# amplab/keystone

Measured on NVIDIA H100. Metric: block-LS fit samples/sec (N=1M, D=64K, k=1K), higher is better.
Workload: dtype f16x2

## Files before the change

### keystone_b200/build.py

```python
from __future__ import annotations

import os
import shutil
import subprocess
import sys

HERE = os.path.dirname(os.path.abspath(__file__))
CSRC = os.path.join(HERE, "csrc")
LIBDIR = os.path.join(HERE, "lib")
LIB = os.path.join(LIBDIR, "libkeystone_b200.so")
SOURCES = ["tc_kernels.cu", "aux_kernels.cu", "solve_kernels.cu", "engine.cu", "bwls.cu", "krr.cu", "lbfgs.cu", "sparse.cu", "logistic.cu", "pca.cu", "fisher.cu", "gmm_fit.cu", "sift.cu", "hog_daisy.cu", "augment.cu", "io.cu"]
HEADERS = ["tc_common.cuh", "kernels.h", "operand_split.cuh", "lbfgs_core.cuh", "engine.h", os.path.join("..", "..", "include", "keystone_b200.h")]
NVCC_FLAGS = [
    "-gencode", "arch=compute_90a,code=sm_90a", "-lineinfo", "-O3", "-std=c++17",
    "-Xcompiler", "-fPIC,-fvisibility=hidden", "-DKS_BUILD",
]


def _nvcc() -> str:
    for cand in (shutil.which("nvcc"), "/usr/local/cuda/bin/nvcc"):
        if cand and os.path.exists(cand):
            return cand
    raise RuntimeError("nvcc not found")


def _stale(target: str, deps) -> bool:
    if not os.path.exists(target):
# ... 31 lines not shown
```

### keystone_b200/csrc/engine.cu

```cuda
#include "engine.h"

#include <cuda_fp16.h>
#include <dlfcn.h>
#include <stdlib.h>
#include <math.h>
#include <string.h>

#include <chrono>
#include <functional>
#include <mutex>
#include <sstream>

namespace ks {

template <class F>
static void load_sym(void* lib, const char* name, F& out, const char* libname) {
  void* s = dlsym(lib, name);
  if (!s) throw KsError{KS_ERR_SOLVER, std::string("symbol ") + name + " missing from " + libname};
  out = reinterpret_cast<F>(s);
}
static void* open_first(const std::vector<const char*>& names) {
  for (const char* n : names) {
    void* h = dlopen(n, RTLD_NOW | RTLD_GLOBAL);
    if (h) return h;
// ... 531 lines not shown
  k.p.vec1 = shift;
  k.p.colsum = colsum;
  k.p.colsumsq = colsumsq;
  k.p.M = static_cast<int>(rows);
  k.p.N = static_cast<int>(cols);
  k.p.K = static_cast<int>(kdepth);
  k.p.flags = (round_out ? 0 : KM_FLAG_NO_ROUND) | (src.kind == 1 ? KM_FLAG_RECT : 0);
  k.p.rect_floor = src.rect_floor;
  k.epi = EPI_COS;
  k.num_sms = (st == c.st2) ? std::max(1, c.num_sms - c.reserve_sms) : c.num_sms;
  if (c.dyn_tiles) k.p.tile_counter = c.next_tile_counter(st);
  KS_CUDA(launch_kmajor(k, st));
  c.launches += 1;
}

const GramTile* gram_tiles(Ctx& c, int b, int kcols, bool with_g, bool with_c, int* num_tiles) {
  std::vector<int> key = {b, kcols, with_g ? 1 : 0, with_c ? 1 : 0};
  auto it = c.tile_cache.find(key);
  std::vector<GramTile> t;
  const int tm = 128, tn = 128;
  const int mb = (b + tm - 1) / tm;
  if (with_g) {
    const int nbk = (b + tn - 1) / tn;
    for (int i = 0; i < mb; ++i)
      for (int j = 0; j < nbk; ++j)
        if ((j + 1) * tn - 1 >= i * tm) t.push_back(GramTile{i, j, 0, 0});
  }
  if (with_c) {
    const int nck = (kcols + tn - 1) / tn;
    for (int i = 0; i < mb; ++i)
      for (int j = 0; j < nck; ++j) t.push_back(GramTile{i, j, 1, 0});
  }
  *num_tiles = static_cast<int>(t.size());
  if (it != c.tile_cache.end()) return it->second->as<GramTile>();
  auto buf = std::make_unique<DevBuf>();
  buf->alloc(sizeof(GramTile) * std::max<size_t>(t.size(), 1));
  KS_CUDA(cudaMemcpyAsync(buf->p, t.data(), sizeof(GramTile) * t.size(), cudaMemcpyHostToDevice, c.st));
  KS_CUDA(cudaStreamSynchronize(c.st));
  const GramTile* p = buf->as<GramTile>();
  c.tile_cache[key] = std::move(buf);
  return p;
}

void launch_gram_block(Ctx& c, const void* slab, int64_t lds, int64_t rows, int b, const void* R, int64_t ldr, int kcols,
                       float* G, int ldg, float* C, int ldc, bool with_g, bool with_c, cudaStream_t st, bool f16,
                       int64_t chunk_rows, const void* slab_lo, const void* R_lo) {
  if (rows <= 0 || b <= 0 || (!with_g && !with_c)) return;
  if (!st) st = c.st;
  const bool split = slab_lo != nullptr;
  if (split && (!f16 || (with_c && !R_lo))) throw KsError{KS_ERR_INVALID, "split Gram operands must be fp16 pairs"};
  GramLaunch g;
  int nt = 0;
  g.f16 = f16 ? 1 : 0;
  g.split = split ? 1 : 0;
  g.tiles = gram_tiles(c, b, kcols, with_g, with_c, &nt);
  g.num_tiles = nt;
  const int stage_rows = split ? 32 : f16 ? 64 : kGramStageRows;
  if (f16) {
    tmap16_or_throw(&g.tmA, slab, rows, b, lds, 64, stage_rows, TMAP_SW128);
    g.tmB0 = g.tmA;
    if (with_c) tmap16_or_throw(&g.tmB1, R, rows, kcols, ldr, 64, stage_rows, TMAP_SW128);
    else g.tmB1 = g.tmA;
    if (split) {
      tmap16_or_throw(&g.tmAlo, slab_lo, rows, b, lds, 64, stage_rows, TMAP_SW128);
      g.tmB0lo = g.tmAlo;
      if (with_c) tmap16_or_throw(&g.tmB1lo, R_lo, rows, kcols, ldr, 64, stage_rows, TMAP_SW128);
      else g.tmB1lo = g.tmAlo;
    }
  } else {
    tmap_or_throw(&g.tmA, static_cast<const float*>(slab), rows, b, lds, kGramStageRows);
// ... 2191 lines not shown
```

### keystone_b200/csrc/engine.h

```cpp
#pragma once
#include <cuda_runtime.h>
#include <cusolverDn.h>
#include <nccl.h>
#include <stdint.h>

#include <map>
#include <memory>
#include <string>
#include <unordered_map>
#include <vector>

#include "../../include/keystone_b200.h"
#include "kernels.h"

namespace ks {

struct KsError {
  int code;
  std::string msg;
};

#define KS_CUDA(call)                                                                                   \
  do {                                                                                                  \
    cudaError_t e__ = (call);                                                                           \
// ... 276 lines not shown
  int64_t ldx3 = 0, ldw3 = 0;
  bool proj_x2 = false;
  DevBuf wcat, wcat_full, bcat;
  int64_t n_rows = 0;
  DevBuf zeros;
};
void make_feat_src(Ctx& c, int64_t features, int64_t x_in, const int64_t* rfs, int32_t n_rfs, FeatSrc& out,
                   int precision = 0);
void prepare_generated_operands(Ctx& c, FeatSrc& out, int precision);
void derive_feat_src(Ctx& c, const FeatSrc& src, Matrix* X, FeatSrc& out, int precision);
void produce_slab(Ctx& c, FeatSrc& src, int64_t c0, int64_t cols, const float* shift, void* slab, int64_t lds,
                  int64_t row_begin, int64_t rows, bool round_out = true, float* colsum = nullptr, cudaStream_t st = nullptr,
                  bool out16 = false, bool x2 = false,
                  void* slab_lo = nullptr,
                  double* colsumsq = nullptr);
const GramTile* gram_tiles(Ctx& c, int b, int kcols, bool with_g, bool with_c, int* num_tiles);
void launch_gram_block(Ctx& c, const void* slab, int64_t lds, int64_t rows, int b, const void* R, int64_t ldr, int kcols,
                       float* G, int ldg, float* C, int ldc, bool with_g, bool with_c, cudaStream_t st = nullptr,
                       bool f16 = false, int64_t chunk_rows = 0,
                       const void* slab_lo = nullptr, const void* R_lo = nullptr);
void launch_update(Ctx& c, const void* slab, int64_t lds, int64_t rows, int b, const void* bop, int64_t ldb, int k,
                   float* out, int64_t ldo, const float* cbias, int epi, bool reduce, cudaStream_t st = nullptr,
                   bool f16 = false, const float* acc_scale_ptr = nullptr,
                   const void* slab_lo = nullptr, const void* bop_lo = nullptr);

int64_t fit_bwls(Ctx& c, FeatSrc& src, Matrix& Y, int bs, int num_iter, double lam, double w, int64_t nf_opt,
                 int precision = KS_PRECISION_TF32);
void launch_set_f64(double* p, double v, cudaStream_t st);
void launch_scale_f64(const double* src, double scale, float* dst, double* dst64, int n, cudaStream_t st);
int64_t fit_lbfgs(Ctx& c, FeatSrc& src, Matrix& Y, bool fit_intercept, int num_corrections, double convergence_tol, int num_iterations,
                  double reg_param, int precision);
// ... 109 lines not shown
```

### keystone_b200/csrc/kernels.h

```cpp
#pragma once
#include <cuda.h>
#include <cuda_runtime.h>
#include <stdint.h>

namespace ks {

static constexpr int kGramStageRows = 32;
static constexpr int kPadCols = 32;

enum { EPI_COS = 0, EPI_UPDATE = 1, EPI_APPLY = 2, EPI_POOL = 3, EPI_RBF = 4 };

struct GramTile {
  int m_blk;
  int n_blk;
  int which;
  int pad;
};
struct GramLaunch {
  CUtensorMap tmA, tmB0, tmB1;
  CUtensorMap tmOut0, tmOut1;
  CUtensorMap tmAlo, tmB0lo, tmB1lo;
  const GramTile* tiles;
  int num_tiles;
  int rows;
  int chunk_rows;
  int n_valid0, n_valid1;
  int f16 = 0;
  int split = 0;
};
enum { KM_FLAG_NO_ROUND = 1, KM_FLAG_REDUCE = 2, KM_FLAG_RECT = 8 };
struct KmParams {
// ... 99 lines not shown
```

### keystone_b200/csrc/solve_kernels.cu

```cuda
#include "kernels.h"

namespace ks {

namespace {
constexpr int TS = 64;
constexpr int U = 16;

__device__ __forceinline__ void dmma(double (&d)[2], double a, double b) {
  asm volatile("mma.sync.aligned.m8n8k4.row.col.f64.f64.f64.f64 {%0, %1}, {%2}, {%3}, {%0, %1};"
               : "+d"(d[0]), "+d"(d[1])
               : "d"(a), "d"(b));
}

template <int NG, bool TRANS>
__device__ __forceinline__ void bulk_dmma(double (&acc)[NG][2], const double* __restrict__ Aptr, size_t lda, int mrow_limit,
                                          const double* Bptr, size_t ldb, const bool (&col_ok)[NG], int k0, int k1, int krow_limit,
                                          int lane) {
  const int m = lane >> 2, kq = lane & 3;
  const bool m_ok = m < mrow_limit;
  if (k0 >= k1) return;
  double a[U], an[U];
  auto load_a = [&](double (&dst)[U], int kb) {
#pragma unroll
    for (int u = 0; u < U; ++u) {
// ... 76 lines not shown
          for (int g = 0; g < NG; ++g) dmma(y[g], a, sV[kk * VP + 8 * g + m]);
        }
      }
#pragma unroll
      for (int g = 0; g < NG; ++g)
#pragma unroll
        for (int e = 0; e < 2; ++e) {
          const int row = r0 + m, col = c0 + 8 * g + 2 * cq + e;
          if (row < n && col < k) B[row + static_cast<size_t>(col) * ld] = y[g][e];
        }
      __syncthreads();
    }
  }
}

__device__ __forceinline__ uint32_t cl_ctarank() {
  uint32_t r;
  asm volatile("mov.u32 %0, %%cluster_ctarank;" : "=r"(r));
  return r;
}
__device__ __forceinline__ uint32_t cl_nctarank() {
  uint32_t r;
  asm volatile("mov.u32 %0, %%cluster_nctarank;" : "=r"(r));
  return r;
}
__device__ __forceinline__ void cl_sync() {
  asm volatile("barrier.cluster.arrive.release.aligned;" ::: "memory");
  asm volatile("barrier.cluster.wait.acquire.aligned;" ::: "memory");
}
__device__ __forceinline__ double ld_dsmem_f64(const double* local_ptr, uint32_t rank) {
  const uint32_t la = static_cast<uint32_t>(__cvta_generic_to_shared(local_ptr));
  uint32_t ra;
  asm("mapa.shared::cluster.u32 %0, %1, %2;" : "=r"(ra) : "r"(la), "r"(rank));
  double v;
  asm volatile("ld.shared::cluster.f64 %0, [%1];" : "=d"(v) : "r"(ra));
  return v;
}

template <bool TRANS>
__device__ __forceinline__ void bulk_dmma_cg(double (&acc)[2], const double* __restrict__ Aptr, size_t lda, int mrow_limit,
                                             const double* Bptr, size_t ldb, bool col_ok, int k0, int k1, int krow_limit, int lane) {
  const int m = lane >> 2, kq = lane & 3;
  const bool m_ok = m < mrow_limit;
  for (int kb = k0; kb < k1; kb += 4 * U) {
    double a[U], b[U];
#pragma unroll
    for (int u = 0; u < U; ++u) {
      const int kk = kb + 4 * u + kq;
// ... 144 lines not shown
```

### keystone_b200/csrc/tc_common.cuh

```cuda
#pragma once
#include <cuda.h>
#include <cuda_fp16.h>
#include <cuda_runtime.h>
#include <stdint.h>

namespace ks {

__device__ unsigned int g_wait_timeout_flag = 0;

static constexpr unsigned long long kWaitBudgetCycles = 6000000000ull;

__device__ __forceinline__ uint32_t smem_u32(const void* p) {
  return static_cast<uint32_t>(__cvta_generic_to_shared(p));
}

__device__ __forceinline__ bool elect_one() {
  uint32_t pred = 0;
  asm volatile(
      "{\n\t"
      ".reg .pred P;\n\t"
      "elect.sync _|P, 0xffffffff;\n\t"
      "selp.u32 %0, 1, 0, P;\n\t"
      "}\n"
      : "=r"(pred));
// ... 8 lines not shown
  asm volatile("mbarrier.init.shared::cta.b64 [%0], %1;" ::"r"(smem_u32(bar)), "r"(count));
}
__device__ __forceinline__ void fence_barrier_init() {
  asm volatile("fence.mbarrier_init.release.cluster;" ::: "memory");
}
__device__ __forceinline__ void fence_proxy_async() {
  asm volatile("fence.proxy.async.shared::cta;" ::: "memory");
}
__device__ __forceinline__ void mbar_arrive_expect_tx(uint64_t* bar, uint32_t bytes) {
  asm volatile("mbarrier.arrive.expect_tx.shared::cta.b64 _, [%0], %1;" ::"r"(smem_u32(bar)), "r"(bytes)
               : "memory");
}
__device__ __forceinline__ void mbar_arrive(uint64_t* bar) {
  asm volatile("mbarrier.arrive.shared::cta.b64 _, [%0];" ::"r"(smem_u32(bar)) : "memory");
}
__device__ __forceinline__ bool mbar_try_wait(uint64_t* bar, uint32_t parity) {
  uint32_t ok;
  asm volatile(
      "{\n\t"
      ".reg .pred P;\n\t"
      "mbarrier.try_wait.parity.shared::cta.b64 P, [%1], %2;\n\t"
      "selp.u32 %0, 1, 0, P;\n\t"
      "}\n"
      : "=r"(ok)
      : "r"(smem_u32(bar)), "r"(parity)
      : "memory");
  return ok != 0;
}
__device__ __forceinline__ void mbar_wait(uint64_t* bar, uint32_t parity) {
  if (mbar_try_wait(bar, parity)) return;
// ... 2 lines not shown
    if (clock64() - t0 > kWaitBudgetCycles) {
      atomicExch(&g_wait_timeout_flag, 1u + (blockIdx.x << 8) + (threadIdx.x >> 5));
      __trap();
    }
  }
}

__device__ __forceinline__ void tma_prefetch_desc(const CUtensorMap* m) {
  asm volatile("prefetch.tensormap [%0];" ::"l"(reinterpret_cast<uint64_t>(m)) : "memory");
}
__device__ __forceinline__ void tma_load_2d(void* smem_dst, const CUtensorMap* m, uint64_t* bar, int32_t c0,
                                            int32_t c1) {
  asm volatile(
      "cp.async.bulk.tensor.2d.shared::cluster.global.mbarrier::complete_tx::bytes [%0], [%1, {%3, %4}], [%2];"
      ::"r"(smem_u32(smem_dst)), "l"(reinterpret_cast<uint64_t>(m)), "r"(smem_u32(bar)), "r"(c0), "r"(c1)
      : "memory");
}

__device__ __forceinline__ void tma_store_2d(const CUtensorMap* m, const void* smem_src, int32_t c0, int32_t c1) {
  asm volatile("cp.async.bulk.tensor.2d.global.shared::cta.bulk_group [%0, {%2, %3}], [%1];" ::"l"(
                   reinterpret_cast<uint64_t>(m)),
               "r"(smem_u32(smem_src)), "r"(c0), "r"(c1)
               : "memory");
}
__device__ __forceinline__ void tma_reduce_add_2d(const CUtensorMap* m, const void* smem_src, int32_t c0, int32_t c1) {
  asm volatile("cp.reduce.async.bulk.tensor.2d.global.shared::cta.add.bulk_group [%0, {%2, %3}], [%1];" ::"l"(
                   reinterpret_cast<uint64_t>(m)),
               "r"(smem_u32(smem_src)), "r"(c0), "r"(c1)
               : "memory");
}
// ... 84 lines not shown
```

### keystone_b200/csrc/tc_kernels.cu

```cuda
#include <type_traits>

#include "tc_common.cuh"
#include "kernels.h"

namespace ks {

static constexpr int kThreads = 384;
static constexpr int kTileM = 128, kTileN = 128;
static constexpr int kStages = 4;
static constexpr int kRawLd = 65;
static constexpr int kRawBytes = 2 * 64 * kRawLd * 4;
static constexpr int kStagingBytes = 8 * 4096;
static constexpr int kVecBytes = 8 * 64 * 4;
static constexpr int kEpiBytes = kStagingBytes + kRawBytes + kVecBytes;
static constexpr int kStageBytes = 32768;
static constexpr int kSmemBytes = kStages * kStageBytes + kEpiBytes + 1024  + 256 ;
static_assert(kSmemBytes <= 227 * 1024, "shared memory per block");

struct SmemLayout {
  uint8_t* stages;
  uint8_t* staging;
  float* raw;
  float* vec;
  uint64_t* full_bar;
// ... 91 lines not shown
    named_bar_sync(1 + g, 128);
    chunk(o, slab, 32 * (w & 1), slab * 64 + 32 * (w >> 1));
  }
}

template <bool F16, bool SPLIT = false>
struct GramCfg {
  static constexpr int PLANES = SPLIT ? 4 : 2;
  static constexpr int SR = SPLIT ? 32 : F16 ? 64 : 32;
  static constexpr int CW = F16 ? 64 : 32;
  static constexpr int NBOX = kTileM / CW;
  static constexpr int BOX_BYTES = SR * 128;
  static constexpr int A_BYTES = NBOX * BOX_BYTES;
  static_assert(PLANES * A_BYTES == kStageBytes, "stage size");
  static_assert(!SPLIT || F16, "split operands are fp16 pairs");
};

template <int BOX_BYTES>
__device__ __forceinline__ uint32_t ld_mn_tf32(const uint8_t* tile, int c, int r) {
  return *reinterpret_cast<const uint32_t*>(tile + (c >> 5) * BOX_BYTES + r * 128 + (((((c & 31) >> 2) ^ (r & 7))) << 4) +
                                            ((c & 3) << 2));
}

template <bool F16, bool SPLIT>
__global__ void __launch_bounds__(kThreads, 1)
gram_tn_kernel(const __grid_constant__ CUtensorMap tmA, const __grid_constant__ CUtensorMap tmB0,
               const __grid_constant__ CUtensorMap tmB1, const __grid_constant__ CUtensorMap tmOut0,
               const __grid_constant__ CUtensorMap tmOut1, const __grid_constant__ CUtensorMap tmAlo,
               const __grid_constant__ CUtensorMap tmB0lo, const __grid_constant__ CUtensorMap tmB1lo,
               const GramTile* __restrict__ tiles, int num_tiles, int rows, int chunk_rows, int n_valid0, int n_valid1) {
  using Cfg = GramCfg<F16, SPLIT>;
  constexpr int SR = Cfg::SR;
  extern __shared__ uint8_t smem_raw[];
  const SmemLayout L = carve_smem(smem_raw);

  const int warp = threadIdx.x >> 5;
  const int lane = threadIdx.x & 31;
  const int wg = warp >> 2;
  const GramTile tile = tiles[blockIdx.x % num_tiles];
  const int chunk = blockIdx.x / num_tiles;
  const int row0 = chunk * chunk_rows;
  const int nrows = min(chunk_rows, rows - row0);
  const int ksteps = (nrows + SR - 1) / SR;
  const int m0 = tile.m_blk * kTileM;
  const int n0 = tile.n_blk * kTileN;
  const CUtensorMap* tmB = tile.which ? &tmB1 : &tmB0;
  const CUtensorMap* tmBlo = tile.which ? &tmB1lo : &tmB0lo;
  const CUtensorMap* tmOut = tile.which ? &tmOut1 : &tmOut0;

  if (threadIdx.x == 0) {
    tma_prefetch_desc(&tmA);
    tma_prefetch_desc(tmB);
    if (SPLIT) {
      tma_prefetch_desc(&tmAlo);
      tma_prefetch_desc(tmBlo);
    }
    tma_prefetch_desc(tmOut);
    for (int s = 0; s < kStages; ++s) {
      mbar_init(&L.full_bar[s], 1);
      mbar_init(&L.empty_bar[s], 8);
    }
    fence_barrier_init();
  }
  __syncthreads();

  if (wg == 0) {
    if (SPLIT) setmaxnreg_dec<40>();
    if (warp == 0 && elect_one()) {
      for (int ks = 0; ks < ksteps; ++ks) {
        const int s = ks % kStages;
        const uint32_t ph = (ks / kStages) & 1;
        mbar_wait(&L.empty_bar[s], ph ^ 1);
        mbar_arrive_expect_tx(&L.full_bar[s], kStageBytes);
        uint8_t* sA = L.stages + s * kStageBytes;
        const int r = row0 + ks * SR;
        const CUtensorMap* maps[4] = {&tmA, SPLIT ? &tmAlo : tmB, tmB, tmBlo};
#pragma unroll
        for (int pl = 0; pl < Cfg::PLANES; ++pl) {
          const int c0 = (pl < Cfg::PLANES / 2) ? m0 : n0;
#pragma unroll
          for (int i = 0; i < Cfg::NBOX; ++i)
            tma_load_2d(sA + pl * Cfg::A_BYTES + i * Cfg::BOX_BYTES, maps[pl], &L.full_bar[s], c0 + Cfg::CW * i, r);
        }
      }
    }
    return;
  }
  if (SPLIT) setmaxnreg_inc<232>();

  const int g = wg - 1;
  const int w = warp & 3;
  float acc[64];
#pragma unroll
  for (int i = 0; i < 64; ++i) acc[i] = 0.f;

  if (SPLIT) {
    float acc_x[64];
#pragma unroll
    for (int i = 0; i < 64; ++i) acc_x[i] = 0.f;
    wgmma_fence_acc(acc);
    wgmma_fence_acc(acc_x);
    int prev = -1;
    for (int ks = 0; ks < ksteps; ++ks) {
      const int s = ks % kStages;
      mbar_wait(&L.full_bar[s], (ks / kStages) & 1);
      const uint32_t st = smem_u32(L.stages + s * kStageBytes);
      const uint32_t sAhi = st + g * Cfg::BOX_BYTES, sAlo = sAhi + Cfg::A_BYTES;
      const uint32_t sBhi = st + 2 * Cfg::A_BYTES, sBlo = st + 3 * Cfg::A_BYTES;
      wgmma_fence();
#pragma unroll
      for (int kk = 0; kk < SR / 16; ++kk)
        wgmma_f16_n128<1, 1>(acc, make_wgmma_desc(sAhi + kk * 2048, Cfg::BOX_BYTES, 1024),
                             make_wgmma_desc(sBhi + kk * 2048, Cfg::BOX_BYTES, 1024), 1);
#pragma unroll
      for (int kk = 0; kk < SR / 16; ++kk) {
        wgmma_f16_n128<1, 1>(acc_x, make_wgmma_desc(sAlo + kk * 2048, Cfg::BOX_BYTES, 1024),
                             make_wgmma_desc(sBhi + kk * 2048, Cfg::BOX_BYTES, 1024), 1);
        wgmma_f16_n128<1, 1>(acc_x, make_wgmma_desc(sAhi + kk * 2048, Cfg::BOX_BYTES, 1024),
                             make_wgmma_desc(sBlo + kk * 2048, Cfg::BOX_BYTES, 1024), 1);
      }
      wgmma_commit();
      if (prev >= 0) {
        wgmma_wait<1>();
        if (lane == 0) mbar_arrive(&L.empty_bar[prev]);
      }
      prev = s;
    }
    wgmma_wait<0>();
    wgmma_fence_acc(acc);
    wgmma_fence_acc(acc_x);
#pragma unroll
    for (int i = 0; i < 64; ++i) acc[i] = __fadd_rn(acc[i], acc_x[i]);
  } else if (F16) {
    wgmma_fence_acc(acc);
    int prev = -1;
    for (int ks = 0; ks < ksteps; ++ks) {
      const int s = ks % kStages;
      mbar_wait(&L.full_bar[s], (ks / kStages) & 1);
      const uint32_t sA = smem_u32(L.stages + s * kStageBytes) + g * Cfg::BOX_BYTES;
// ... 68 lines not shown
    }
  };
  auto chunk_fn = [&](float (&o)[32], int, int r_off, int c_off) {
    const int col = n0 + c_off;
    if (col >= n_valid) return;
    if (lane == 0) bulk_wait_read0();
    __syncwarp();
    stage_row_sw128(buf, lane, o);
    fence_proxy_async();
    __syncwarp();
    if (lane == 0) {
      tma_reduce_add_2d(tmOut, buf, col, m0 + 64 * g + r_off);
      bulk_commit();
    }
  };
  epilogue_slabs(raw, g, w, lane, to_raw, chunk_fn);
  if (lane == 0) bulk_wait0();
}

__device__ __forceinline__ float cos_reduced(float x) {
  const float kInv2Pi = 0.15915494309189535f;
  const float k2PiHi = 6.2831854820251465f;
  const float k2PiLo = -1.7484555314695172e-7f;
  const float kMagic = 12582912.0f;
  const float k = __fadd_rn(__fmaf_rn(x, kInv2Pi, kMagic), -kMagic);
  float r = fmaf(-k, k2PiHi, x);
  r = fmaf(-k, k2PiLo, r);
  return __cosf(r);
}

__device__ __forceinline__ void stage_row_f16(uint8_t* buf, int lane, const float (&o)[32]) {
  uint4* row = reinterpret_cast<uint4*>(buf + lane * 64);
// ... 185 lines not shown
                   const __grid_constant__ CUtensorMap tmAlo, const __grid_constant__ CUtensorMap tmBlo, KmParams p) {
  static_assert(!SPLIT || F16, "split operands are fp16 pairs");
  constexpr bool ASYNC = km_async(EPI);
  static_assert(!(ASYNC && SPLIT), "the split update keeps its in-place epilogue");
  constexpr int ROW_BYTES = SPLIT ? 64 : 128;
  constexpr int BK = ROW_BYTES / (F16 ? 2 : 4);
  constexpr int A_BYTES = kTileM * ROW_BYTES;
  extern __shared__ uint8_t smem_raw[];
  const KmSmem L = carve_km_smem<ASYNC>(smem_raw);

  const int warp = threadIdx.x >> 5;
  const int lane = threadIdx.x & 31;
  const int wg = warp >> 2;
  const int m_tiles = (p.M + kTileM - 1) / kTileM;
  const int n_tiles = (p.N + kTileN - 1) / kTileN;
  const int total_tiles = m_tiles * n_tiles;
  const int ksteps = (p.K + BK - 1) / BK;

  if (threadIdx.x == 0) {
    tma_prefetch_desc(&tmA);
    tma_prefetch_desc(&tmB);
    if (SPLIT) {
      tma_prefetch_desc(&tmAlo);
      tma_prefetch_desc(&tmBlo);
    }
    tma_prefetch_desc(&tmOut);
    for (int s = 0; s < kStages; ++s) {
      mbar_init(&L.full_bar[s], 1);
      mbar_init(&L.empty_bar[s], 8);
    }
    for (int r = 0; r < 8; ++r) mbar_init(&L.ring_bar[r], 1);
    if (ASYNC) {
      mbar_init(L.tile_full, 256);
      mbar_init(L.tile_empty, 32 * kEpiWarps);
    }
    fence_barrier_init();
  }
  __syncthreads();

  if (ASYNC && ((warp >= 1 && warp < 4) || warp >= 12)) {
    const int e = warp < 4 ? warp - 1 : warp - 9;
    const int rb = e & 3, cb = 2 * (e >> 2);
    uint8_t* sbuf = L.staging + e * 4096;
    const float ascale = p.acc_scale_ptr ? __ldg(p.acc_scale_ptr) * p.acc_scale : p.acc_scale;
    uint32_t staged = 0;
    for (uint32_t tl = 0;; ++tl) {
      mbar_wait(L.tile_full, tl & 1);
      const int t = *L.tile_id;
      if (t < 0) break;
      const int m0 = (t / n_tiles) * kTileM;
      const int n0 = (t % n_tiles) * kTileN;
      {
        named_bar_sync(1, 32 * kEpiWarps);
// ... 14 lines not shown
        }
        float o[32];
#pragma unroll
        for (int i = 0; i < 32; ++i) o[i] = lds_f32(src + 4 * (32 * c + i));
        if (k == 1) mbar_arrive(L.tile_empty);
        km_chunk<EPI, OUT16>(p, &tmOut, &tmOut2, o, L.vec + 64 * c, sbuf, staged & 1, m0 + 32 * rb, col0, lane, ascale);
        ++staged;
      }
    }
    if (lane == 0) bulk_wait0();
    return;
  }
  if (wg == 0) {
    if (warp == 0 && elect_one()) {
      uint32_t it = 0, tl = 0;
      int next = p.tile_counter ? atomicAdd(p.tile_counter, 1) : static_cast<int>(blockIdx.x);
      for (;; ++tl) {
        const int t = next < total_tiles ? next : -1;
        L.tile_ring[tl & 7] = t;
        mbar_arrive(&L.ring_bar[tl & 7]);
        if (t < 0) break;
        next = p.tile_counter ? atomicAdd(p.tile_counter, 1) : t + static_cast<int>(gridDim.x);
        const int m0 = (t / n_tiles) * kTileM;
        const int n0 = (t % n_tiles) * kTileN;
        for (int ks = 0; ks < ksteps; ++ks, ++it) {
          const int s = it % kStages;
          const uint32_t ph = (it / kStages) & 1;
          mbar_wait(&L.empty_bar[s], ph ^ 1);
          mbar_arrive_expect_tx(&L.full_bar[s], kStageBytes);
          uint8_t* sA = L.stages + s * kStageBytes;
          if (SPLIT) {
            tma_load_2d(sA, &tmA, &L.full_bar[s], ks * BK, m0);
            tma_load_2d(sA + A_BYTES, &tmAlo, &L.full_bar[s], ks * BK, m0);
            tma_load_2d(sA + 2 * A_BYTES, &tmB, &L.full_bar[s], ks * BK, n0);
            tma_load_2d(sA + 3 * A_BYTES, &tmBlo, &L.full_bar[s], ks * BK, n0);
          } else {
            tma_load_2d(sA, &tmA, &L.full_bar[s], ks * BK, m0);
            tma_load_2d(sA + A_BYTES, &tmB, &L.full_bar[s], ks * BK, n0);
          }
        }
      }
    }
    return;
  }

  const int g = wg - 1;
  const int w = warp & 3;
  float* raw = L.raw + g * 64 * kRawLd;
  float* vs = L.vec + (warp - 4) * 64;
  uint8_t* sbuf = L.staging + (warp - 4) * 4096;
  const float ascale = p.acc_scale_ptr ? __ldg(p.acc_scale_ptr) * p.acc_scale : p.acc_scale;
  uint32_t it = 0;
  for (uint32_t tl = 0;; ++tl) {
    mbar_wait(&L.ring_bar[tl & 7], (tl >> 3) & 1);
    const int t = L.tile_ring[tl & 7];
    if (ASYNC && t < 0) {
      mbar_wait(L.tile_empty, (tl & 1) ^ 1);
      if (threadIdx.x == 128) *L.tile_id = -1;
      mbar_arrive(L.tile_full);
      return;
    }
    if (t < 0) break;
    const int m0 = (t / n_tiles) * kTileM;
    const int n0 = (t % n_tiles) * kTileN;

    float acc[64];
#pragma unroll
    for (int i = 0; i < 64; ++i) acc[i] = 0.f;
    if (SPLIT) {
      float acc_x[64];
#pragma unroll
      for (int i = 0; i < 64; ++i) acc_x[i] = 0.f;
      wgmma_fence_acc(acc);
      wgmma_fence_acc(acc_x);
      int prev = -1;
      for (int ks = 0; ks < ksteps; ++ks, ++it) {
        const int s = it % kStages;
        mbar_wait(&L.full_bar[s], (it / kStages) & 1);
        const uint32_t sAhi = smem_u32(L.stages + s * kStageBytes) + g * 64 * ROW_BYTES;
        const uint32_t sAlo = sAhi + A_BYTES;
        const uint32_t sBhi = smem_u32(L.stages + s * kStageBytes) + 2 * A_BYTES, sBlo = sBhi + A_BYTES;
        wgmma_fence();
#pragma unroll
        for (int kk = 0; kk < 2; ++kk)
          wgmma_f16_n128<0, 0>(acc, make_wgmma_desc<2>(sAhi + kk * 32, 16, 512), make_wgmma_desc<2>(sBhi + kk * 32, 16, 512), 1);
#pragma unroll
        for (int kk = 0; kk < 2; ++kk) {
          wgmma_f16_n128<0, 0>(acc_x, make_wgmma_desc<2>(sAlo + kk * 32, 16, 512), make_wgmma_desc<2>(sBhi + kk * 32, 16, 512), 1);
          wgmma_f16_n128<0, 0>(acc_x, make_wgmma_desc<2>(sAhi + kk * 32, 16, 512), make_wgmma_desc<2>(sBlo + kk * 32, 16, 512), 1);
        }
        wgmma_commit();
        if (prev >= 0) {
          wgmma_wait<1>();
          if (lane == 0) mbar_arrive(&L.empty_bar[prev]);
        }
        prev = s;
      }
      wgmma_wait<0>();
      wgmma_fence_acc(acc);
      wgmma_fence_acc(acc_x);
      if (prev >= 0 && lane == 0) mbar_arrive(&L.empty_bar[prev]);
#pragma unroll
      for (int i = 0; i < 64; ++i) acc[i] = __fadd_rn(acc[i], acc_x[i]);
    } else {
      wgmma_fence_acc(acc);
      int prev = -1;
      for (int ks = 0; ks < ksteps; ++ks, ++it) {
        const int s = it % kStages;
        mbar_wait(&L.full_bar[s], (it / kStages) & 1);
        const uint32_t sA = smem_u32(L.stages + s * kStageBytes) + g * 64 * 128;
        const uint32_t sB = smem_u32(L.stages + s * kStageBytes) + A_BYTES;
        wgmma_fence();
#pragma unroll
        for (int kk = 0; kk < 4; ++kk) {
          const uint64_t ad = make_wgmma_desc(sA + kk * 32, 16, 1024);
          const uint64_t bd = make_wgmma_desc(sB + kk * 32, 16, 1024);
// ... 20 lines not shown
      continue;
    }
    auto to_raw = [&](float* rw, int slab) { wgmma_acc_to_raw(acc, rw, slab, w, lane); };
    auto chunk_fn = [&](float (&o)[32], int slab, int r_off, int c_off) {
      const int col0 = n0 + c_off;
      if (col0 >= p.N) return;
      __syncwarp();
      vs[lane] = (p.vec0 && col0 + lane < p.N) ? __ldg(p.vec0 + col0 + lane) : 0.f;
      vs[32 + lane] = (p.vec1 && col0 + lane < p.N) ? __ldg(p.vec1 + col0 + lane) : 0.f;
      __syncwarp();
      km_chunk<EPI, OUT16>(p, &tmOut, &tmOut2, o, vs, sbuf, slab & 1, m0 + 64 * g + r_off, col0, lane, ascale);
    };
    epilogue_slabs(raw, g, w, lane, to_raw, chunk_fn);
  }
  if (lane == 0) bulk_wait0();
}

typedef CUresult (*PFN_encodeTiled)(CUtensorMap*, CUtensorMapDataType, cuuint32_t, void*, const cuuint64_t*,
                                    const cuuint64_t*, const cuuint32_t*, const cuuint32_t*, CUtensorMapInterleave,
                                    CUtensorMapSwizzle, CUtensorMapL2promotion, CUtensorMapFloatOOBfill);

static PFN_encodeTiled get_encode_fn() {
  static PFN_encodeTiled fn = nullptr;
  if (!fn) {
    void* p = nullptr;
    cudaDriverEntryPointQueryResult qres;
    if (cudaGetDriverEntryPoint("cuTensorMapEncodeTiled", &p, cudaEnableDefault, &qres) != cudaSuccess ||
        qres != cudaDriverEntryPointSuccess)
      return nullptr;
    fn = reinterpret_cast<PFN_encodeTiled>(p);
// ... 20 lines not shown
                  const_cast<void*>(base), dims, strides, box, estr, CU_TENSOR_MAP_INTERLEAVE_NONE, sw,
                  CU_TENSOR_MAP_L2_PROMOTION_L2_256B, CU_TENSOR_MAP_FLOAT_OOB_FILL_NONE);
  return r == CUDA_SUCCESS ? 0 : -static_cast<int>(r) - 1000;
}

template <typename K>
static cudaError_t set_smem_attr_once(K kern, bool& done, int bytes = kSmemBytes) {
  if (!done) {
    cudaError_t e = cudaFuncSetAttribute(kern, cudaFuncAttributeMaxDynamicSharedMemorySize, bytes);
    if (e != cudaSuccess) return e;
    done = true;
  }
  return cudaSuccess;
}

template <bool F16, bool SPLIT>
static cudaError_t launch_gram_t(const GramLaunch& g, cudaStream_t st) {
  if (g.chunk_rows % GramCfg<F16, SPLIT>::SR != 0) return cudaErrorInvalidValue;
  auto kern = gram_tn_kernel<F16, SPLIT>;
  static bool attr_done = false;
  cudaError_t e = set_smem_attr_once(kern, attr_done);
  if (e != cudaSuccess) return e;
  const int chunks = (g.rows + g.chunk_rows - 1) / g.chunk_rows;
  const unsigned grid = static_cast<unsigned>(chunks) * static_cast<unsigned>(g.num_tiles);
  if (grid == 0) return cudaSuccess;
  kern<<<grid, kThreads, kSmemBytes, st>>>(g.tmA, g.tmB0, g.tmB1, g.tmOut0, g.tmOut1, SPLIT ? g.tmAlo : g.tmA, SPLIT ? g.tmB0lo : g.tmB0,
                                           SPLIT ? g.tmB1lo : g.tmB1, g.tiles, g.num_tiles, g.rows, g.chunk_rows, g.n_valid0, g.n_valid1);
  return cudaGetLastError();
}

cudaError_t launch_gram(const GramLaunch& g, cudaStream_t st) {
  if (g.split) return g.f16 ? launch_gram_t<true, true>(g, st) : cudaErrorInvalidValue;
  return g.f16 ? launch_gram_t<true, false>(g, st) : launch_gram_t<false, false>(g, st);
}

template <int EPI, bool F16, int OUT16, bool SPLIT = false>
static cudaError_t launch_km_t(const KmLaunch& k, cudaStream_t st) {
  auto kern = gemm_kmajor_kernel<EPI, F16, OUT16, SPLIT>;
  static bool attr_done = false;
  cudaError_t e = set_smem_attr_once(kern, attr_done, km_smem_bytes(EPI));
  if (e != cudaSuccess) return e;
  const int m_tiles = (k.p.M + kTileM - 1) / kTileM;
  const int n_tiles = (k.p.N + kTileN - 1) / kTileN;
  const long long total = static_cast<long long>(m_tiles) * n_tiles;
  if (total == 0) return cudaSuccess;
  const unsigned grid = static_cast<unsigned>(total < k.num_sms ? total : k.num_sms);
  kern<<<grid, km_threads(EPI), km_smem_bytes(EPI), st>>>(k.tmA, k.tmB, k.tmOut, OUT16 == 2 ? k.tmOut2 : k.tmOut, SPLIT ? k.tmAlo : k.tmA,
                                           SPLIT ? k.tmBlo : k.tmB, k.p);
  return cudaGetLastError();
}

cudaError_t launch_kmajor(const KmLaunch& k, cudaStream_t st) {
  if (k.split) return (k.f16 && k.epi == EPI_UPDATE) ? launch_km_t<EPI_UPDATE, true, 0, true>(k, st) : cudaErrorInvalidValue;
  if (k.epi == EPI_POOL) return k.f16 ? launch_km_t<EPI_POOL, true, 0>(k, st) : cudaErrorInvalidValue;
  if (k.epi == EPI_RBF) return (k.f16 && k.out16 == 2) ? launch_km_t<EPI_RBF, true, 2>(k, st) : cudaErrorInvalidValue;
  if (k.f16 && k.epi == EPI_APPLY) return launch_km_t<EPI_APPLY, true, 0>(k, st);
  if (k.f16 && k.epi == EPI_UPDATE) return launch_km_t<EPI_UPDATE, true, 0>(k, st);
  if (k.out16 == 2 && k.epi == EPI_COS) return k.f16 ? launch_km_t<EPI_COS, true, 2>(k, st) : cudaErrorInvalidValue;
  if (k.out16 && k.f16 && k.epi == EPI_COS) return launch_km_t<EPI_COS, true, 1>(k, st);
  if (k.f16 && k.epi == EPI_COS) return launch_km_t<EPI_COS, true, 0>(k, st);
// ... 17 lines not shown
```

Before: 298,000.

## Pair split-operand Gram and update kernels in 2-CTA clusters with TMA multicast

Launches the split (hi/lo fp16) Gram and k-major update kernels as 2-CTA clusters. CTA pairs share an operand plane: each CTA fetches one half of the shared operand and multicasts it to both, which roughly halves global/L2 traffic for that operand. Odd tiles are padded with idle partner tiles. Stage release signals both CTAs' empty barriers, so the two CTAs now advance in lockstep and pay cluster syncs and remote mbarrier arrives. The update kernel also drops dynamic tile scheduling in favour of a static per-pair stride.

```diff
diff --git a/keystone_b200/build.py b/keystone_b200/build.py
--- a/keystone_b200/build.py
+++ b/keystone_b200/build.py
@@ -10,7 +10,7 @@
 LIBDIR = os.path.join(HERE, "lib")
 LIB = os.path.join(LIBDIR, "libkeystone_b200.so")
 SOURCES = ["tc_kernels.cu", "aux_kernels.cu", "solve_kernels.cu", "engine.cu", "bwls.cu", "krr.cu", "lbfgs.cu", "sparse.cu", "logistic.cu", "pca.cu", "fisher.cu", "gmm_fit.cu", "sift.cu", "hog_daisy.cu", "augment.cu", "io.cu"]
-HEADERS = ["tc_common.cuh", "kernels.h", "operand_split.cuh", "lbfgs_core.cuh", "engine.h", os.path.join("..", "..", "include", "keystone_b200.h")]
+HEADERS = ["tc_common.cuh", "cluster.cuh", "kernels.h", "operand_split.cuh", "lbfgs_core.cuh", "engine.h", os.path.join("..", "..", "include", "keystone_b200.h")]
 NVCC_FLAGS = [
     "-gencode", "arch=compute_90a,code=sm_90a", "-lineinfo", "-O3", "-std=c++17",
     "-Xcompiler", "-fPIC,-fvisibility=hidden", "-DKS_BUILD",
diff --git a/keystone_b200/csrc/cluster.cuh b/keystone_b200/csrc/cluster.cuh
--- /dev/null
+++ b/keystone_b200/csrc/cluster.cuh
@@ -0,0 +1,26 @@
+#pragma once
+#include <stdint.h>
+
+namespace ks {
+
+__device__ __forceinline__ uint32_t cl_ctarank() {
+  uint32_t r;
+  asm volatile("mov.u32 %0, %%cluster_ctarank;" : "=r"(r));
+  return r;
+}
+__device__ __forceinline__ uint32_t cl_nctarank() {
+  uint32_t r;
+  asm volatile("mov.u32 %0, %%cluster_nctarank;" : "=r"(r));
+  return r;
+}
+__device__ __forceinline__ void cl_sync() {
+  asm volatile("barrier.cluster.arrive.release.aligned;" ::: "memory");
+  asm volatile("barrier.cluster.wait.acquire.aligned;" ::: "memory");
+}
+__device__ __forceinline__ uint32_t cl_map_shared(uint32_t local_addr, uint32_t rank) {
+  uint32_t ra;
+  asm("mapa.shared::cluster.u32 %0, %1, %2;" : "=r"(ra) : "r"(local_addr), "r"(rank));
+  return ra;
+}
+
+}
diff --git a/keystone_b200/csrc/engine.cu b/keystone_b200/csrc/engine.cu
--- a/keystone_b200/csrc/engine.cu
+++ b/keystone_b200/csrc/engine.cu
@@ -569,22 +569,47 @@
   c.launches += 1;
 }
 
-const GramTile* gram_tiles(Ctx& c, int b, int kcols, bool with_g, bool with_c, int* num_tiles) {
-  std::vector<int> key = {b, kcols, with_g ? 1 : 0, with_c ? 1 : 0};
+static void pair_tiles(std::vector<GramTile>& t, int mb, int nb, int which, bool upper) {
+  std::vector<GramTile> left;
+  for (int i = 0; i < mb; ++i) {
+    int j = upper ? i : 0;
+    for (; j + 1 < nb; j += 2) {
+      t.push_back(GramTile{i, j, which, 0});
+      t.push_back(GramTile{i, j + 1, which, 0});
+    }
+    if (j < nb) left.push_back(GramTile{i, j, which, GRAM_SHARE_B});
+  }
+  for (size_t q = 0; q + 1 < left.size(); q += 2) {
+    t.push_back(left[q]);
+    t.push_back(left[q + 1]);
+  }
+  if (left.size() % 2) {
+    const GramTile lone = left.back();
+    t.push_back(lone);
+    t.push_back(GramTile{lone.m_blk, lone.n_blk, which, GRAM_SHARE_B | GRAM_IDLE});
+  }
+}
+
+const GramTile* gram_tiles(Ctx& c, int b, int kcols, bool with_g, bool with_c, bool split, int* num_tiles) {
+  std::vector<int> key = {b, kcols, with_g ? 1 : 0, with_c ? 1 : 0, split ? 1 : 0};
   auto it = c.tile_cache.find(key);
   std::vector<GramTile> t;
   const int tm = 128, tn = 128;
   const int mb = (b + tm - 1) / tm;
   if (with_g) {
     const int nbk = (b + tn - 1) / tn;
-    for (int i = 0; i < mb; ++i)
-      for (int j = 0; j < nbk; ++j)
-        if ((j + 1) * tn - 1 >= i * tm) t.push_back(GramTile{i, j, 0, 0});
+    if (split) pair_tiles(t, mb, nbk, 0, true);
+    else
+      for (int i = 0; i < mb; ++i)
+        for (int j = 0; j < nbk; ++j)
+          if ((j + 1) * tn - 1 >= i * tm) t.push_back(GramTile{i, j, 0, 0});
   }
   if (with_c) {
     const int nck = (kcols + tn - 1) / tn;
-    for (int i = 0; i < mb; ++i)
-      for (int j = 0; j < nck; ++j) t.push_back(GramTile{i, j, 1, 0});
+    if (split) pair_tiles(t, mb, nck, 1, false);
+    else
+      for (int i = 0; i < mb; ++i)
+        for (int j = 0; j < nck; ++j) t.push_back(GramTile{i, j, 1, 0});
   }
   *num_tiles = static_cast<int>(t.size());
   if (it != c.tile_cache.end()) return it->second->as<GramTile>();
@@ -608,7 +633,7 @@
   int nt = 0;
   g.f16 = f16 ? 1 : 0;
   g.split = split ? 1 : 0;
-  g.tiles = gram_tiles(c, b, kcols, with_g, with_c, &nt);
+  g.tiles = gram_tiles(c, b, kcols, with_g, with_c, split, &nt);
   g.num_tiles = nt;
   const int stage_rows = split ? 32 : f16 ? 64 : kGramStageRows;
   if (f16) {
diff --git a/keystone_b200/csrc/engine.h b/keystone_b200/csrc/engine.h
--- a/keystone_b200/csrc/engine.h
+++ b/keystone_b200/csrc/engine.h
@@ -314,7 +314,7 @@
                   bool out16 = false, bool x2 = false,
                   void* slab_lo = nullptr,
                   double* colsumsq = nullptr);
-const GramTile* gram_tiles(Ctx& c, int b, int kcols, bool with_g, bool with_c, int* num_tiles);
+const GramTile* gram_tiles(Ctx& c, int b, int kcols, bool with_g, bool with_c, bool split, int* num_tiles);
 void launch_gram_block(Ctx& c, const void* slab, int64_t lds, int64_t rows, int b, const void* R, int64_t ldr, int kcols,
                        float* G, int ldg, float* C, int ldc, bool with_g, bool with_c, cudaStream_t st = nullptr,
                        bool f16 = false, int64_t chunk_rows = 0,
diff --git a/keystone_b200/csrc/kernels.h b/keystone_b200/csrc/kernels.h
--- a/keystone_b200/csrc/kernels.h
+++ b/keystone_b200/csrc/kernels.h
@@ -10,11 +10,12 @@
 
 enum { EPI_COS = 0, EPI_UPDATE = 1, EPI_APPLY = 2, EPI_POOL = 3, EPI_RBF = 4 };
 
+enum { GRAM_SHARE_B = 1, GRAM_IDLE = 2 };
 struct GramTile {
   int m_blk;
   int n_blk;
   int which;
-  int pad;
+  int pair;
 };
 struct GramLaunch {
   CUtensorMap tmA, tmB0, tmB1;
diff --git a/keystone_b200/csrc/solve_kernels.cu b/keystone_b200/csrc/solve_kernels.cu
--- a/keystone_b200/csrc/solve_kernels.cu
+++ b/keystone_b200/csrc/solve_kernels.cu
@@ -1,3 +1,4 @@
+#include "cluster.cuh"
 #include "kernels.h"
 
 namespace ks {
@@ -114,24 +115,8 @@
   }
 }
 
-__device__ __forceinline__ uint32_t cl_ctarank() {
-  uint32_t r;
-  asm volatile("mov.u32 %0, %%cluster_ctarank;" : "=r"(r));
-  return r;
-}
-__device__ __forceinline__ uint32_t cl_nctarank() {
-  uint32_t r;
-  asm volatile("mov.u32 %0, %%cluster_nctarank;" : "=r"(r));
-  return r;
-}
-__device__ __forceinline__ void cl_sync() {
-  asm volatile("barrier.cluster.arrive.release.aligned;" ::: "memory");
-  asm volatile("barrier.cluster.wait.acquire.aligned;" ::: "memory");
-}
 __device__ __forceinline__ double ld_dsmem_f64(const double* local_ptr, uint32_t rank) {
-  const uint32_t la = static_cast<uint32_t>(__cvta_generic_to_shared(local_ptr));
-  uint32_t ra;
-  asm("mapa.shared::cluster.u32 %0, %1, %2;" : "=r"(ra) : "r"(la), "r"(rank));
+  const uint32_t ra = cl_map_shared(static_cast<uint32_t>(__cvta_generic_to_shared(local_ptr)), rank);
   double v;
   asm volatile("ld.shared::cluster.f64 %0, [%1];" : "=d"(v) : "r"(ra));
   return v;
diff --git a/keystone_b200/csrc/tc_common.cuh b/keystone_b200/csrc/tc_common.cuh
--- a/keystone_b200/csrc/tc_common.cuh
+++ b/keystone_b200/csrc/tc_common.cuh
@@ -3,6 +3,8 @@
 #include <cuda_fp16.h>
 #include <cuda_runtime.h>
 #include <stdint.h>
+
+#include "cluster.cuh"
 
 namespace ks {
 
@@ -46,6 +48,9 @@
 __device__ __forceinline__ void mbar_arrive(uint64_t* bar) {
   asm volatile("mbarrier.arrive.shared::cta.b64 _, [%0];" ::"r"(smem_u32(bar)) : "memory");
 }
+__device__ __forceinline__ void mbar_arrive_remote(uint32_t cluster_addr) {
+  asm volatile("mbarrier.arrive.shared::cluster.b64 _, [%0];" ::"r"(cluster_addr) : "memory");
+}
 __device__ __forceinline__ bool mbar_try_wait(uint64_t* bar, uint32_t parity) {
   uint32_t ok;
   asm volatile(
@@ -78,6 +83,14 @@
   asm volatile(
       "cp.async.bulk.tensor.2d.shared::cluster.global.mbarrier::complete_tx::bytes [%0], [%1, {%3, %4}], [%2];"
       ::"r"(smem_u32(smem_dst)), "l"(reinterpret_cast<uint64_t>(m)), "r"(smem_u32(bar)), "r"(c0), "r"(c1)
+      : "memory");
+}
+__device__ __forceinline__ void tma_load_2d_mc(void* smem_dst, const CUtensorMap* m, uint64_t* bar, int32_t c0, int32_t c1,
+                                               uint16_t cta_mask) {
+  asm volatile(
+      "cp.async.bulk.tensor.2d.shared::cluster.global.mbarrier::complete_tx::bytes.multicast::cluster [%0], [%1, {%4, %5}], [%2], "
+      "%3;" ::"r"(smem_u32(smem_dst)),
+      "l"(reinterpret_cast<uint64_t>(m)), "r"(smem_u32(bar)), "h"(cta_mask), "r"(c0), "r"(c1)
       : "memory");
 }
 
diff --git a/keystone_b200/csrc/tc_kernels.cu b/keystone_b200/csrc/tc_kernels.cu
--- a/keystone_b200/csrc/tc_kernels.cu
+++ b/keystone_b200/csrc/tc_kernels.cu
@@ -1,3 +1,4 @@
+#include <algorithm>
 #include <type_traits>
 
 #include "tc_common.cuh"
@@ -129,6 +130,7 @@
   static constexpr int A_BYTES = NBOX * BOX_BYTES;
   static_assert(PLANES * A_BYTES == kStageBytes, "stage size");
   static_assert(!SPLIT || F16, "split operands are fp16 pairs");
+  static_assert(!SPLIT || NBOX == 2, "each CTA of a pair fetches one box of each shared plane");
 };
 
 template <int BOX_BYTES>
@@ -152,8 +154,12 @@
   const int warp = threadIdx.x >> 5;
   const int lane = threadIdx.x & 31;
   const int wg = warp >> 2;
-  const GramTile tile = tiles[blockIdx.x % num_tiles];
-  const int chunk = blockIdx.x / num_tiles;
+  const uint32_t rank = SPLIT ? cl_ctarank() : 0;
+  const int pairs = num_tiles / 2;
+  const GramTile tile = SPLIT ? tiles[2 * ((blockIdx.x >> 1) % pairs) + rank] : tiles[blockIdx.x % num_tiles];
+  const int chunk = SPLIT ? (blockIdx.x >> 1) / pairs : blockIdx.x / num_tiles;
+  const bool idle = SPLIT && (tile.pair & GRAM_IDLE);
+  const bool share_b = SPLIT && (tile.pair & GRAM_SHARE_B);
   const int row0 = chunk * chunk_rows;
   const int nrows = min(chunk_rows, rows - row0);
   const int ksteps = (nrows + SR - 1) / SR;
@@ -173,11 +179,12 @@
     tma_prefetch_desc(tmOut);
     for (int s = 0; s < kStages; ++s) {
       mbar_init(&L.full_bar[s], 1);
-      mbar_init(&L.empty_bar[s], 8);
+      mbar_init(&L.empty_bar[s], SPLIT ? 16 : 8);
     }
     fence_barrier_init();
   }
-  __syncthreads();
+  if (SPLIT) cl_sync();
+  else __syncthreads();
 
   if (wg == 0) {
     if (SPLIT) setmaxnreg_dec<40>();
@@ -186,18 +193,27 @@
         const int s = ks % kStages;
         const uint32_t ph = (ks / kStages) & 1;
         mbar_wait(&L.empty_bar[s], ph ^ 1);
-        mbar_arrive_expect_tx(&L.full_bar[s], kStageBytes);
+        mbar_arrive_expect_tx(&L.full_bar[s], idle ? kStageBytes / 2 : kStageBytes);
         uint8_t* sA = L.stages + s * kStageBytes;
         const int r = row0 + ks * SR;
         const CUtensorMap* maps[4] = {&tmA, SPLIT ? &tmAlo : tmB, tmB, tmBlo};
 #pragma unroll
         for (int pl = 0; pl < Cfg::PLANES; ++pl) {
           const int c0 = (pl < Cfg::PLANES / 2) ? m0 : n0;
+          if (SPLIT && (pl >= Cfg::PLANES / 2) == share_b) {
+            tma_load_2d_mc(sA + pl * Cfg::A_BYTES + rank * Cfg::BOX_BYTES, maps[pl], &L.full_bar[s], c0 + Cfg::CW * rank, r, 0x3);
+            continue;
+          }
+          if (idle) continue;
 #pragma unroll
           for (int i = 0; i < Cfg::NBOX; ++i)
             tma_load_2d(sA + pl * Cfg::A_BYTES + i * Cfg::BOX_BYTES, maps[pl], &L.full_bar[s], c0 + Cfg::CW * i, r);
         }
       }
+    }
+    if (SPLIT) {
+      __syncwarp();
+      cl_sync();
     }
     return;
   }
@@ -215,10 +231,19 @@
     for (int i = 0; i < 64; ++i) acc_x[i] = 0.f;
     wgmma_fence_acc(acc);
     wgmma_fence_acc(acc_x);
+    const uint32_t peer_empty = cl_map_shared(smem_u32(L.empty_bar), rank ^ 1);
+    auto release = [&](int s) {
+      mbar_arrive(&L.empty_bar[s]);
+      mbar_arrive_remote(peer_empty + 8 * s);
+    };
     int prev = -1;
     for (int ks = 0; ks < ksteps; ++ks) {
       const int s = ks % kStages;
       mbar_wait(&L.full_bar[s], (ks / kStages) & 1);
+      if (idle) {
+        if (lane == 0) release(s);
+        continue;
+      }
       const uint32_t st = smem_u32(L.stages + s * kStageBytes);
       const uint32_t sAhi = st + g * Cfg::BOX_BYTES, sAlo = sAhi + Cfg::A_BYTES;
       const uint32_t sBhi = st + 2 * Cfg::A_BYTES, sBlo = st + 3 * Cfg::A_BYTES;
@@ -237,7 +262,7 @@
       wgmma_commit();
       if (prev >= 0) {
         wgmma_wait<1>();
-        if (lane == 0) mbar_arrive(&L.empty_bar[prev]);
+        if (lane == 0) release(prev);
       }
       prev = s;
     }
@@ -336,8 +361,12 @@
       bulk_commit();
     }
   };
-  epilogue_slabs(raw, g, w, lane, to_raw, chunk_fn);
+  if (!idle) epilogue_slabs(raw, g, w, lane, to_raw, chunk_fn);
   if (lane == 0) bulk_wait0();
+  if (SPLIT) {
+    __syncwarp();
+    cl_sync();
+  }
 }
 
 __device__ __forceinline__ float cos_reduced(float x) {
@@ -553,8 +582,12 @@
   const int wg = warp >> 2;
   const int m_tiles = (p.M + kTileM - 1) / kTileM;
   const int n_tiles = (p.N + kTileN - 1) / kTileN;
-  const int total_tiles = m_tiles * n_tiles;
+  const int n_pairs = (n_tiles + 1) / 2;
+  const uint32_t rank = SPLIT ? (blockIdx.x & 1) : 0;
+  const int total_tiles = SPLIT ? m_tiles * n_pairs : m_tiles * n_tiles;
   const int ksteps = (p.K + BK - 1) / BK;
+  auto tile_m0 = [&](int t) { return (t / (SPLIT ? n_pairs : n_tiles)) * kTileM; };
+  auto tile_n0 = [&](int t) { return SPLIT ? (2 * (t % n_pairs) + static_cast<int>(rank)) * kTileN : (t % n_tiles) * kTileN; };
 
   if (threadIdx.x == 0) {
     tma_prefetch_desc(&tmA);
@@ -566,7 +599,7 @@
     tma_prefetch_desc(&tmOut);
     for (int s = 0; s < kStages; ++s) {
       mbar_init(&L.full_bar[s], 1);
-      mbar_init(&L.empty_bar[s], 8);
+      mbar_init(&L.empty_bar[s], SPLIT ? 16 : 8);
     }
     for (int r = 0; r < 8; ++r) mbar_init(&L.ring_bar[r], 1);
     if (ASYNC) {
@@ -575,7 +608,8 @@
     }
     fence_barrier_init();
   }
-  __syncthreads();
+  if (SPLIT) cl_sync();
+  else __syncthreads();
 
   if (ASYNC && ((warp >= 1 && warp < 4) || warp >= 12)) {
     const int e = warp < 4 ? warp - 1 : warp - 9;
@@ -620,32 +654,41 @@
   if (wg == 0) {
     if (warp == 0 && elect_one()) {
       uint32_t it = 0, tl = 0;
-      int next = p.tile_counter ? atomicAdd(p.tile_counter, 1) : static_cast<int>(blockIdx.x);
+      int next = SPLIT ? static_cast<int>(blockIdx.x >> 1)
+                       : p.tile_counter ? atomicAdd(p.tile_counter, 1) : static_cast<int>(blockIdx.x);
       for (;; ++tl) {
         const int t = next < total_tiles ? next : -1;
         L.tile_ring[tl & 7] = t;
         mbar_arrive(&L.ring_bar[tl & 7]);
         if (t < 0) break;
-        next = p.tile_counter ? atomicAdd(p.tile_counter, 1) : t + static_cast<int>(gridDim.x);
-        const int m0 = (t / n_tiles) * kTileM;
-        const int n0 = (t % n_tiles) * kTileN;
+        next = SPLIT ? t + static_cast<int>(gridDim.x >> 1)
+                     : p.tile_counter ? atomicAdd(p.tile_counter, 1) : t + static_cast<int>(gridDim.x);
+        const int m0 = tile_m0(t);
+        const int n0 = tile_n0(t);
+        const bool idle = SPLIT && n0 >= p.N;
         for (int ks = 0; ks < ksteps; ++ks, ++it) {
           const int s = it % kStages;
           const uint32_t ph = (it / kStages) & 1;
           mbar_wait(&L.empty_bar[s], ph ^ 1);
-          mbar_arrive_expect_tx(&L.full_bar[s], kStageBytes);
+          mbar_arrive_expect_tx(&L.full_bar[s], idle ? kStageBytes / 2 : kStageBytes);
           uint8_t* sA = L.stages + s * kStageBytes;
           if (SPLIT) {
-            tma_load_2d(sA, &tmA, &L.full_bar[s], ks * BK, m0);
-            tma_load_2d(sA + A_BYTES, &tmAlo, &L.full_bar[s], ks * BK, m0);
-            tma_load_2d(sA + 2 * A_BYTES, &tmB, &L.full_bar[s], ks * BK, n0);
-            tma_load_2d(sA + 3 * A_BYTES, &tmBlo, &L.full_bar[s], ks * BK, n0);
+            if (rank == 0) tma_load_2d_mc(sA, &tmA, &L.full_bar[s], ks * BK, m0, 0x3);
+            else tma_load_2d_mc(sA + A_BYTES, &tmAlo, &L.full_bar[s], ks * BK, m0, 0x3);
+            if (!idle) {
+              tma_load_2d(sA + 2 * A_BYTES, &tmB, &L.full_bar[s], ks * BK, n0);
+              tma_load_2d(sA + 3 * A_BYTES, &tmBlo, &L.full_bar[s], ks * BK, n0);
+            }
           } else {
             tma_load_2d(sA, &tmA, &L.full_bar[s], ks * BK, m0);
             tma_load_2d(sA + A_BYTES, &tmB, &L.full_bar[s], ks * BK, n0);
           }
         }
       }
+    }
+    if (SPLIT) {
+      __syncwarp();
+      cl_sync();
     }
     return;
   }
@@ -667,8 +710,21 @@
       return;
     }
     if (t < 0) break;
-    const int m0 = (t / n_tiles) * kTileM;
-    const int n0 = (t % n_tiles) * kTileN;
+    const int m0 = tile_m0(t);
+    const int n0 = tile_n0(t);
+
+    auto release = [&](int s) {
+      mbar_arrive(&L.empty_bar[s]);
+      if (SPLIT) mbar_arrive_remote(cl_map_shared(smem_u32(&L.empty_bar[s]), rank ^ 1));
+    };
+    if (SPLIT && n0 >= p.N) {
+      for (int ks = 0; ks < ksteps; ++ks, ++it) {
+        const int s = it % kStages;
+        mbar_wait(&L.full_bar[s], (it / kStages) & 1);
+        if (lane == 0) release(s);
+      }
+      continue;
+    }
 
     float acc[64];
 #pragma unroll
@@ -698,14 +754,14 @@
         wgmma_commit();
         if (prev >= 0) {
           wgmma_wait<1>();
-          if (lane == 0) mbar_arrive(&L.empty_bar[prev]);
+          if (lane == 0) release(prev);
         }
         prev = s;
       }
       wgmma_wait<0>();
       wgmma_fence_acc(acc);
       wgmma_fence_acc(acc_x);
-      if (prev >= 0 && lane == 0) mbar_arrive(&L.empty_bar[prev]);
+      if (prev >= 0 && lane == 0) release(prev);
 #pragma unroll
       for (int i = 0; i < 64; ++i) acc[i] = __fadd_rn(acc[i], acc_x[i]);
     } else {
@@ -756,6 +812,10 @@
     epilogue_slabs(raw, g, w, lane, to_raw, chunk_fn);
   }
   if (lane == 0) bulk_wait0();
+  if (SPLIT) {
+    __syncwarp();
+    cl_sync();
+  }
 }
 
 typedef CUresult (*PFN_encodeTiled)(CUtensorMap*, CUtensorMapDataType, cuuint32_t, void*, const cuuint64_t*,
@@ -806,6 +866,38 @@
   return cudaSuccess;
 }
 
+static cudaLaunchConfig_t pair_config(unsigned grid, int smem, cudaStream_t st, cudaLaunchAttribute* attr) {
+  cudaLaunchConfig_t cfg = {};
+  cfg.gridDim = dim3(grid);
+  cfg.blockDim = dim3(kThreads);
+  cfg.dynamicSmemBytes = static_cast<size_t>(smem);
+  cfg.stream = st;
+  attr[0].id = cudaLaunchAttributeClusterDimension;
+  attr[0].val.clusterDim.x = 2;
+  attr[0].val.clusterDim.y = 1;
+  attr[0].val.clusterDim.z = 1;
+  cfg.attrs = attr;
+  cfg.numAttrs = 1;
+  return cfg;
+}
+template <typename K, typename... Args>
+static cudaError_t launch_pairs(K kern, unsigned grid, int smem, cudaStream_t st, Args... args) {
+  cudaLaunchAttribute attr[1];
+  const cudaLaunchConfig_t cfg = pair_config(grid, smem, st, attr);
+  const cudaError_t e = cudaLaunchKernelEx(&cfg, kern, args...);
+  return e != cudaSuccess ? e : cudaGetLastError();
+}
+template <typename K>
+static cudaError_t resident_pairs(K kern, int smem, int num_sms, int* pairs) {
+  cudaLaunchAttribute attr[1];
+  const cudaLaunchConfig_t cfg = pair_config(static_cast<unsigned>(std::max(2, num_sms & ~1)), smem, nullptr, attr);
+  int n = 0;
+  const cudaError_t e = cudaOccupancyMaxActiveClusters(&n, kern, &cfg);
+  if (e != cudaSuccess) return e;
+  *pairs = std::max(1, std::min(n, num_sms / 2));
+  return cudaSuccess;
+}
+
 template <bool F16, bool SPLIT>
 static cudaError_t launch_gram_t(const GramLaunch& g, cudaStream_t st) {
   if (g.chunk_rows % GramCfg<F16, SPLIT>::SR != 0) return cudaErrorInvalidValue;
@@ -816,6 +908,11 @@
   const int chunks = (g.rows + g.chunk_rows - 1) / g.chunk_rows;
   const unsigned grid = static_cast<unsigned>(chunks) * static_cast<unsigned>(g.num_tiles);
   if (grid == 0) return cudaSuccess;
+  if (SPLIT) {
+    if (g.num_tiles % 2 != 0) return cudaErrorInvalidValue;
+    return launch_pairs(kern, grid, kSmemBytes, st, g.tmA, g.tmB0, g.tmB1, g.tmOut0, g.tmOut1, g.tmAlo, g.tmB0lo, g.tmB1lo, g.tiles,
+                        g.num_tiles, g.rows, g.chunk_rows, g.n_valid0, g.n_valid1);
+  }
   kern<<<grid, kThreads, kSmemBytes, st>>>(g.tmA, g.tmB0, g.tmB1, g.tmOut0, g.tmOut1, SPLIT ? g.tmAlo : g.tmA, SPLIT ? g.tmB0lo : g.tmB0,
                                            SPLIT ? g.tmB1lo : g.tmB1, g.tiles, g.num_tiles, g.rows, g.chunk_rows, g.n_valid0, g.n_valid1);
   return cudaGetLastError();
@@ -836,6 +933,17 @@
   const int n_tiles = (k.p.N + kTileN - 1) / kTileN;
   const long long total = static_cast<long long>(m_tiles) * n_tiles;
   if (total == 0) return cudaSuccess;
+  if (SPLIT) {
+    if (k.p.tile_counter) return cudaErrorInvalidValue;
+    static int fit = 0;
+    if (!fit) {
+      e = resident_pairs(kern, km_smem_bytes(EPI), k.num_sms, &fit);
+      if (e != cudaSuccess) return e;
+    }
+    const long long pairs = static_cast<long long>(m_tiles) * ((n_tiles + 1) / 2);
+    const unsigned grid = 2u * static_cast<unsigned>(std::min<long long>(pairs, std::min(fit, std::max(1, k.num_sms / 2))));
+    return launch_pairs(kern, grid, km_smem_bytes(EPI), st, k.tmA, k.tmB, k.tmOut, k.tmOut, k.tmAlo, k.tmBlo, k.p);
+  }
   const unsigned grid = static_cast<unsigned>(total < k.num_sms ? total : k.num_sms);
   kern<<<grid, km_threads(EPI), km_smem_bytes(EPI), st>>>(k.tmA, k.tmB, k.tmOut, OUT16 == 2 ? k.tmOut2 : k.tmOut, SPLIT ? k.tmAlo : k.tmA,
                                            SPLIT ? k.tmBlo : k.tmB, k.p);
```

After: 310,300 (median of 6 runs). 1.04x the previous value.
